# LenShustek/readtape

Hardware: AMD Instinct MI355X
Metric: Msamples/sec (all tracks) 9-trk TBIN (higher is better)
Workload: dtype i16/f32; 1 GPU; C2: synthetic 9-track 800 BPI NRZI, 781.25 kHz, 1 parmset; rows_per_gpu=101799450, rows_total=101799450, bytes_per_gpu=1832390100, parmsets=1

## Files before the change

### readtape_amd/csrc/rtfe_api.hip

```cpp
#include <hip/hip_runtime.h>

#include <limits.h>
#include <math.h>
#include <stdarg.h>
#include <stdio.h>
#include <stdlib.h>
#include <string.h>

#include <mutex>

#include "rt_frontend.h"
#include "rtfe_device.h"

#include "rtfe_sift.hip"
#include "rtfe_kernels.hip"
#include "rtfe_zeros.hip"
#include "rtfe_diffz.hip"
#include "rtfe_ww.hip"
#include "rtfe_gain.hip"
#include "rtfe_dense.hip"
#include "rtfe_pack.hip"
#include "rtfe_csv.hip"

namespace rtfe {
// ... 345 lines not shown
      fprintf(stderr, "rtfe: peak path %d, k_sift LDS %d (halo %d/%d rows, slots %d bytes, %d vectors per thread)\n", d.peak_path, d.pk_lds, d.pk_hl, d.pk_hr, d.pk_slot, sf_nv(d));
      for (int sidx = 0; sidx < d.nscreens; ++sidx) fprintf(stderr, "rtfe: screen %d W %d rise_i %d minpk_i %d sure_i %d\n", sidx, d.screen[sidx].W, d.screen[sidx].rise_i, d.screen[sidx].minpk_i, d.screen[sidx].sure_i); }
   hipDeviceProp_t prop;
   int dev = 0;
   if (hipGetDevice(&dev) != hipSuccess || hipGetDeviceProperties(&prop, dev) != hipSuccess) { delete h; return fail(-20, "no HIP device"); }
   h->num_cus = prop.multiProcessorCount;
   if (hipMalloc(&h->d_dev, sizeof(DevCfg)) != hipSuccess) { delete h; return fail(-21, "hipMalloc failed"); }
   if (hipMemcpy(h->d_dev, &d, sizeof(DevCfg), hipMemcpyHostToDevice) != hipSuccess) { (void)hipFree(h->d_dev); delete h; return fail(-22, "hipMemcpy failed"); }
   raise_dynamic_lds(reinterpret_cast<const void *>(k_decode), h->lds_bytes);
   h->zeros_kernel = getenv("RTFE_ZEROS_KERNEL") ? atoi(getenv("RTFE_ZEROS_KERNEL")) != 0 : 1;
   h->diffz_kernel = getenv("RTFE_DIFFZ_KERNEL") ? atoi(getenv("RTFE_DIFFZ_KERNEL")) != 0 : 1;
   if (!(d.find_zeros && d.differentiate) || d.mode == RTFE_WW) h->diffz_kernel = 0;
   h->side = nullptr; h->overlap = getenv("RTFE_OVERLAP") ? atoi(getenv("RTFE_OVERLAP")) != 0 : 1;
   h->graphs = getenv("RTFE_GRAPHS") ? atoi(getenv("RTFE_GRAPHS")) != 0 : 0;
   memset(h->gcache, 0, sizeof h->gcache); h->gstamp = 0;
   h->bursts_wpr = getenv("RTFE_BURSTS_WPR") ? atoi(getenv("RTFE_BURSTS_WPR")) : 0;
   h->ds_order = getenv("RTFE_DS_ORDER") ? atoi(getenv("RTFE_DS_ORDER")) : 1;
   h->dchain_wgs = getenv("RTFE_DCHAIN_WGS") ? atoi(getenv("RTFE_DCHAIN_WGS")) : 16;
   h->prep_wgs = getenv("RTFE_PREP_WGS") ? atoi(getenv("RTFE_PREP_WGS")) : 32;
   h->prep_run = getenv("RTFE_PREP_RUN") ? atoi(getenv("RTFE_PREP_RUN")) : 8;
   if (h->prep_run < 1 || h->prep_run > kPrepMaxRun) h->prep_run = 8;
   h->work_cap = getenv("RTFE_WORK_CAP") ? atoll(getenv("RTFE_WORK_CAP")) : -1;
   h->ccap_max = getenv("RTFE_CCAP") ? atoll(getenv("RTFE_CCAP")) : 0;
   h->dense_stop = getenv("RTFE_DENSE_STOP") ? atoi(getenv("RTFE_DENSE_STOP")) : 99;
   h->dseg_wgs = getenv("RTFE_DSEG_WGS") ? atoi(getenv("RTFE_DSEG_WGS")) : 0;
   h->dseg_threads = getenv("RTFE_DSEG_THREADS") ? atoi(getenv("RTFE_DSEG_THREADS")) : 0;
   h->seg_cap = getenv("RTFE_SEG_CAP") ? atoll(getenv("RTFE_SEG_CAP")) : 0;
   h->peak_stop = getenv("RTFE_PEAK_STOP") ? atoi(getenv("RTFE_PEAK_STOP")) : 99;
   h->sift_wgs = getenv("RTFE_SIFT_WGS") ? atoi(getenv("RTFE_SIFT_WGS")) : 0;
   h->sift_generic = getenv("RTFE_SIFT_GENERIC") != nullptr;
   h->sift_per_screen = !(getenv("RTFE_SIFT_PER_SCREEN") && atoi(getenv("RTFE_SIFT_PER_SCREEN")) == 0);
   h->dseg_generic = getenv("RTFE_DSEG_GENERIC") != nullptr;
   if (d.invert || d.maxskew > 0 || d.ntrks < 2 || d.zc_peak_i < 1 || d.zc_peak_i > 32767 || !d.zc_parallel) h->zeros_kernel = 0;
   if (d.peak_path) {
      raise_dynamic_lds(reinterpret_cast<const void *>(sf_kernel(sf_wmax(d), sf_threads(d), sf_nv(d))), d.pk_lds);
      for (int sc = 0; sc < kMaxScreens; ++sc) h->sfs_occ[sc] = 0;
      if (sf_special(h)) for (int sc = 0; sc < d.nscreens; ++sc) {
         raise_dynamic_lds(reinterpret_cast<const void *>(sf_special_sc(h, sc)), sfs_lds_sc(d, sc));
         int nb = 0;
         if (hipOccupancyMaxActiveBlocksPerMultiprocessor(&nb, reinterpret_cast<const void *>(sf_special_sc(h, sc)), sfs_threads(d), (size_t)sfs_lds_sc(d, sc)) == hipSuccess && nb >= 1) h->sfs_occ[sc] = nb; } }
   if (d.dense_path) raise_dynamic_lds(reinterpret_cast<const void *>(ds_kernel(h)), (int)ds_lds_layout(d.ntrks, d.halo_rows, d.ds_pad + kDsTile + kDsRight, d.ds_up).total + 64);
   (void)hipGetLastError();
   if (getenv("RTFE_VERBOSE") && d.peak_path) {
      int nb = -1;
      const sfs_kernel_t sfs = sf_special(h);
      const int thr = sfs ? sfs_threads(d) : sf_threads(d), lds = sfs ? sfs_lds(d) : d.pk_lds;
      (void)hipOccupancyMaxActiveBlocksPerMultiprocessor(&nb, sfs ? reinterpret_cast<const void *>(sfs) : reinterpret_cast<const void *>(sf_kernel(sf_wmax(d), sf_threads(d), sf_nv(d))), thr, (size_t)lds);
      fprintf(stderr, "rtfe: k_sift%s %d threads, %d bytes of LDS: %d workgroups per CU (occupancy API), %d CUs\n", sfs ? "_s" : "", thr, lds, nb, h->num_cus); }
   *out = h;
   return 0; }

constexpr int kTimingRing = 64;
static_assert(kTimingRing <= 64, "rtfe_handle::ev_ran holds 64 sets");
static void timing_free(rtfe_handle *h) {
   if (!h->ev0) return;
   for (int r = 0; r < kTimingRing; ++r) for (int i = 0; i < kNumKernels; ++i) { (void)hipEventDestroy(h->ev0[r][i]); (void)hipEventDestroy(h->ev1[r][i]); }
   delete[] h->ev0; delete[] h->ev1; h->ev0 = nullptr; h->ev1 = nullptr; }

extern "C" int rtfe_set_timing(rtfe_handle *h, int enable) {
   if (!h) return fail(-1, "null argument");
   if (enable && !h->timing) {
      h->ev0 = new hipEvent_t[kTimingRing][12]; h->ev1 = new hipEvent_t[kTimingRing][12];
      for (int r = 0; r < kTimingRing; ++r) for (int i = 0; i < kNumKernels; ++i)
      {
         const bool ok0 = hipEventCreate(&h->ev0[r][i]) == hipSuccess;
         const bool ok1 = ok0 && hipEventCreate(&h->ev1[r][i]) == hipSuccess;
         if (!ok1) {
            if (ok0) (void)hipEventDestroy(h->ev0[r][i]);
            for (int r2 = 0; r2 <= r; ++r2) for (int i2 = 0; i2 < (r2 < r ? kNumKernels : i); ++i2) { (void)hipEventDestroy(h->ev0[r2][i2]); (void)hipEventDestroy(h->ev1[r2][i2]); }
            delete[] h->ev0; delete[] h->ev1; h->ev0 = nullptr; h->ev1 = nullptr;
            return fail(-40, "hipEventCreate failed"); } }
      h->ev_next = 0; h->ev_pending = 0; }
   if (!enable && h->timing) timing_free(h);
   h->timing = enable != 0;
   return 0; }

extern "C" int rtfe_kernel_ms(rtfe_handle *h, float *out) {
   if (!h || !out || !h->timing) return fail(-41, "timing is not enabled");
   const int n = h->ev_pending < kTimingRing ? h->ev_pending : kTimingRing;
   for (int i = 0; i < kNumKernels; ++i) out[i] = 0;
   for (int k = 0; k < n; ++k) {
      const int r = ((h->ev_next - 1 - k) % kTimingRing + kTimingRing) % kTimingRing;
      for (int i = 0; i < kNumKernels; ++i) {
         float ms = 0;
         if (hipEventSynchronize(h->ev1[r][i]) != hipSuccess) return fail(-42, "hipEventSynchronize failed");
         if (hipEventElapsedTime(&ms, h->ev0[r][i], h->ev1[r][i]) != hipSuccess) return fail(-43, "hipEventElapsedTime failed");
         if ((h->ev_ran[r] >> i) & 1u) out[i] += ms; } }
   h->ev_pending = 0;
   return n; }

extern "C" void rtfe_destroy(rtfe_handle *h) {
   if (!h) return;
   if (h->timing) timing_free(h);
   drop_graphs(h);
   if (h->side) { (void)hipEventDestroy(h->ev_fork); (void)hipEventDestroy(h->ev_join); (void)hipEventDestroy(h->ev_fork2); (void)hipEventDestroy(h->ev_join2); (void)hipStreamDestroy(h->side); }
   (void)hipFree(h->d_dev);
   delete h; }

extern "C" int rtfe_pkww_width(const rtfe_handle *h, int parmset) {
   return (h && parmset >= 0 && parmset < h->dev.nparm) ? h->dev.parm[parmset].W : -1; }

constexpr int kBrRoundsMax = 1024;

extern "C" int64_t rtfe_max_bursts(const rtfe_handle *h, int64_t nrows) {
   return (nrows / kChunkRows) / h->dev.gap_chunks + 4; }

struct WsLayout {
   long long nwords, max_bursts, ptiles, dtiles;
   long long ccap, seg_cap, work_cap; int hard_cap;
   size_t scratch, qwords, rtot, ctl, dir, chain, pool, hard, ovf, qtile, tstart, crec, eref, extra, cst, segs, gfire, work, dead, slot, total; };

static size_t align256(size_t x) { return (x + 255) & ~(size_t)255; }

static WsLayout ws_layout(const rtfe_handle *h, int64_t nrows) {
   const DevCfg &d = h->dev;
   const bool pk = d.peak_path != 0, ds = d.dense_path != 0;
   const size_t nlists = (size_t)d.nscreens * d.ntrks, nchains = (size_t)d.nparm * d.ntrks;
   WsLayout L;
   L.nwords = ((nrows / kChunkRows + 1) + 63) / 64 + 1;
   L.max_bursts = rtfe_max_bursts(h, nrows);
   L.ptiles = (nrows + kSfTile - 1) / kSfTile;
   L.dtiles = (nrows + kDsTile - 1) / kDsTile;
   L.ccap = L.ptiles * (d.pk_slot / 8 + 1) + 64;
   if (h->ccap_max > 0 && h->ccap_max < L.ccap) L.ccap = h->ccap_max;
   const long long sift_wgs = L.ptiles < (long long)h->num_cus * 8 ? L.ptiles : (long long)h->num_cus * 8;
   const long long hard = L.ptiles * d.nscreens * d.ntrks * 2 + 4096 + sift_wgs * 4 * kSfHardChunk * d.nscreens;
   L.hard_cap = (int)(hard > 0x3fffffffll ? 0x3fffffffll : hard);
   L.seg_cap = 0;
   if (pk) L.seg_cap = h->seg_cap >= 1 ? h->seg_cap
                                       : (L.ccap / d.pk_seg_recs + 1) * d.nscreens * d.ntrks * (d.nparm < 2 ? 1 : 2) + L.max_bursts * d.nparm * d.ntrks + 64;
   size_t off = 0;
   auto take = [&off](bool on, size_t bytes) { const size_t at = off; if (on) off = align256(off + bytes); return at; };
   L.scratch = 0;
   L.qwords = kScratchBytes;
   L.rtot = L.qwords + (size_t)L.nwords * 8;
   off = align256(L.rtot + (size_t)kBrRoundsMax * 4);
   L.ctl = take(true, (size_t)L.max_bursts * sizeof(BurstCtl));
   L.dir = take(pk, (size_t)(L.ptiles + 1) * nlists * sizeof(PeakDir));
   L.chain = take(pk, (size_t)L.max_bursts * nchains * sizeof(float));
   L.pool = take(pk, (size_t)L.ptiles * nlists * (size_t)d.pk_slot);
   L.hard = take(pk, (size_t)L.hard_cap * sizeof(SfHard));
   L.ovf = take(pk, (size_t)L.hard_cap * kSfOvfBytes);
   L.qtile = take(pk, (size_t)L.ptiles * 2);
   L.tstart = take(pk, ((size_t)L.ptiles + 2 * ((size_t)(L.ptiles + 1023) / 1024) + 2) * nlists * 4);
   L.crec = take(pk, (size_t)L.ccap * nlists * sizeof(CRec));
   L.eref = take(pk, (size_t)L.ccap * nlists * 8);
   L.extra = take(pk, (size_t)L.ptiles * nlists * 4);
   L.cst = take(pk, (size_t)L.max_bursts * nchains * sizeof(ChainSt));
   L.segs = take(pk, (size_t)L.seg_cap * sizeof(GsSeg));
   L.gfire = take(pk, (size_t)L.seg_cap * (size_t)(d.pk_seg_recs > 0 ? d.pk_seg_recs : 0) * 4);
   L.work = L.gfire;
   L.work_cap = (long long)((off - L.gfire) / 8);
   if (h->work_cap >= 0 && h->work_cap < L.work_cap) L.work_cap = h->work_cap;
   if (L.work_cap > 0x7ffffe00ll) L.work_cap = 0x7ffffe00ll;
   L.dead = take(ds, (size_t)L.dtiles * d.nscreens);
   L.slot = take(ds, (size_t)L.dtiles * kDsJ * d.nuset * d.ntrks * (size_t)d.ds_slot + 256);
   L.total = off + 256;
   return L; }

extern "C" size_t rtfe_workspace_bytes(const rtfe_handle *h, int64_t nrows) { return ws_layout(h, nrows).total; }

extern "C" int64_t rtfe_event_capacity(const rtfe_handle *h, int64_t nrows) {
   const double per_track = (double)nrows * h->dev.cap_frac + 128.0 * (double)rtfe_max_bursts(h, nrows) + (double)kMarginRows;
   return (int64_t)(per_track * h->dev.nparm * h->dev.ntrks) + 4096; }

struct WsView {
   BurstScratch *scratch; unsigned long long *qwords; uint32_t *rtot; BurstCtl *ctl;
   PeakDir *dir; float *chain; unsigned char *pool; SfHard *hard; unsigned char *ovf; uint16_t *qtile;
   uint32_t *tstart, *ctotc, *coff, *ctot;
   CRec *crec; uint2 *eref; int *extra; ChainSt *cst; GsSeg *segs; float *gfire; unsigned long long *work;
   unsigned char *dead, *slot; };

template <class T> static T *ws_at(void *ws, size_t off) { return reinterpret_cast<T *>(static_cast<char *>(ws) + off); }

static WsView ws_view(const rtfe_handle *h, const WsLayout &L, void *ws) {
   WsView w;
   w.scratch = ws_at<BurstScratch>(ws, L.scratch); w.qwords = ws_at<unsigned long long>(ws, L.qwords); w.rtot = ws_at<uint32_t>(ws, L.rtot); w.ctl = ws_at<BurstCtl>(ws, L.ctl);
   w.dir = ws_at<PeakDir>(ws, L.dir); w.chain = ws_at<float>(ws, L.chain); w.pool = ws_at<unsigned char>(ws, L.pool); w.hard = ws_at<SfHard>(ws, L.hard);
   w.ovf = ws_at<unsigned char>(ws, L.ovf); w.qtile = ws_at<uint16_t>(ws, L.qtile);
   const size_t nlists = h->dev.peak_path ? (size_t)h->dev.nscreens * h->dev.ntrks : 0, nsc = (size_t)(L.ptiles + 1023) / 1024;
   w.tstart = ws_at<uint32_t>(ws, L.tstart); w.ctotc = w.tstart + (size_t)L.ptiles * nlists; w.coff = w.ctotc + nsc * nlists; w.ctot = w.coff + nsc * nlists;
   w.crec = ws_at<CRec>(ws, L.crec); w.eref = ws_at<uint2>(ws, L.eref); w.extra = ws_at<int>(ws, L.extra); w.cst = ws_at<ChainSt>(ws, L.cst);
   w.segs = ws_at<GsSeg>(ws, L.segs); w.gfire = ws_at<float>(ws, L.gfire); w.work = ws_at<unsigned long long>(ws, L.work);
   w.dead = ws_at<unsigned char>(ws, L.dead); w.slot = ws_at<unsigned char>(ws, L.slot);
   return w; }

static int launch_check(const char *what) {
   hipError_t e = hipGetLastError();
   if (e != hipSuccess) return fail(-30, "%s: %s", what, hipGetErrorString(e));
   return 0; }

static void ensure_side(rtfe_handle *h) {
   if (h->side || !h->overlap) return;
   int pr_least = 0, pr_greatest = 0;
   (void)hipDeviceGetStreamPriorityRange(&pr_least, &pr_greatest);
   if (hipStreamCreateWithPriority(&h->side, hipStreamNonBlocking, pr_greatest) != hipSuccess) { (void)hipGetLastError(); h->side = nullptr; h->overlap = 0; }
   else { (void)hipEventCreateWithFlags(&h->ev_fork, hipEventDisableTiming); (void)hipEventCreateWithFlags(&h->ev_join, hipEventDisableTiming);
          (void)hipEventCreateWithFlags(&h->ev_fork2, hipEventDisableTiming); (void)hipEventCreateWithFlags(&h->ev_join2, hipEventDisableTiming); } }

struct ScanArgs {
   const int16_t *d_rows; int64_t nrows, own_rows, row_base; int first_is_tape_start;
   void *d_workspace; size_t workspace_bytes;
   rtfe_burst *d_bursts; int64_t max_bursts; int32_t *d_nbursts;
   uint32_t *d_counts; rtfe_event *d_events; int64_t event_capacity; void *stream; };

static void graph_key(const ScanArgs &a, unsigned long long key[13]) {
   auto u = [](auto v) { return (unsigned long long)(uintptr_t)v; };
   const unsigned long long k[13] = {u(a.d_rows), u(a.nrows), u(a.own_rows), u(a.row_base), u(a.first_is_tape_start), u(a.d_workspace), u(a.workspace_bytes),
                                     u(a.d_bursts), u(a.max_bursts), u(a.d_nbursts), u(a.d_counts), u(a.d_events), u(a.event_capacity)};
   memcpy(key, k, sizeof k); }

struct Scan {
   rtfe_handle *h; const DevCfg &d; const ScanArgs &a; hipStream_t st; WsLayout L; WsView w;
   long long nrows, row_base, nchunks, maxb;
   int evset; bool ran[kNumKernels];
   void t0s(int k, hipStream_t s) { ran[k] = true; if (h->timing) (void)hipEventRecord(h->ev0[evset][k], s); }
   void t1s(int k, hipStream_t s) { if (h->timing) (void)hipEventRecord(h->ev1[evset][k], s); }
   void t0(int k) { t0s(k, st); }
   void t1(int k) { t1s(k, st); }
   void skip_rest() {
      unsigned mask = 0;
      for (int k = 0; k < kNumKernels; ++k) if (ran[k]) mask |= 1u << k;
      if (h->timing) h->ev_ran[evset] = mask;
      for (int k = 0; k < kNumKernels; ++k) if (!ran[k]) { t0(k); t1(k); } }
   void launch_bursts(hipStream_t s) {
      const int wpr_env = h->bursts_wpr;
      const int wpr = (wpr_env >= 1 && wpr_env <= kBrWords) ? wpr_env : kBrWords;
      const long long rounds = (L.nwords + wpr - 1) / wpr;
      if ((wpr_env > 0 || rounds >= 3) && rounds <= kBrRoundsMax && d.debug != 5) {
         hipLaunchKernelGGL(k_bursts_cnt, dim3((unsigned)rounds), dim3(1024), 0, s, (const unsigned long long *)w.qwords, L.nwords, nchunks, wpr, d.gap_chunks, a.first_is_tape_start, maxb, w.rtot);
         hipLaunchKernelGGL(k_bursts_emit, dim3((unsigned)rounds), dim3(1024), 0, s, (const unsigned long long *)w.qwords, L.nwords, nchunks, nrows, wpr, d.gap_chunks, a.first_is_tape_start, a.d_bursts, maxb, (const uint32_t *)w.rtot);
         hipLaunchKernelGGL(k_bursts_tail, dim3(1), dim3(1024), 0, s, (int)rounds, (const uint32_t *)w.rtot, nrows, (long long)a.own_rows, d.ntrks, d.gap_chunks,
                            d.cap_frac, d.nparm, (long long)a.event_capacity, a.d_bursts, maxb, w.scratch, a.d_nbursts); }
      else
         hipLaunchKernelGGL(k_bursts, dim3(1), dim3(1024), 0, s, (const unsigned long long *)w.qwords, L.nwords, nchunks, nrows, (long long)a.own_rows, d.ntrks,
                            d.gap_chunks, a.first_is_tape_start, d.cap_frac, d.nparm, (long long)a.event_capacity, a.d_bursts, maxb, w.scratch, a.d_nbursts, d.debug == 5 ? 1 : 0); }
   void launch_zones(hipStream_t s) {
      hipLaunchKernelGGL(k_zones, dim3(h->num_cus * 8), dim3(64), 0, s, h->d_dev, a.d_rows, nrows, (const rtfe_burst *)a.d_bursts, (const BurstScratch *)w.scratch, w.ctl);
      if (d.invert)
         hipLaunchKernelGGL(k_rails, dim3(h->num_cus * 8), dim3(64), 0, s, h->d_dev, a.d_rows, nrows, (const rtfe_burst *)a.d_bursts, (const BurstScratch *)w.scratch, w.ctl); }
   void launch_decode(int mode) {
      const DecodePlan dp = decode_plan(h);
      t0(kTDecode);
      hipLaunchKernelGGL(k_decode, dim3(h->num_cus * dp.per_cu), dim3(dp.threads), h->lds_bytes, st, h->d_dev, a.d_rows, nrows,
                         row_base, a.d_bursts, w.scratch, a.d_counts, a.d_events, 0xffffffffu, 0, 0, mode, w.ctl);
      t1(kTDecode); }
   void launch_sift() {
      t0(kTSift);
      const sfs_kernel_t sfs = sf_special(h);
      const int pthreads = sfs ? sfs_threads(d) : sf_threads(d), plds = sfs ? sfs_lds(d) : d.pk_lds;
      int spc = lds_wgs_per_cu(plds, 512, 32 / (pthreads / 64));
      if (h->sift_wgs >= 1 && h->sift_wgs < spc) spc = h->sift_wgs;
      if (spc < 1) spc = 1;
      long long pgrid = (long long)h->num_cus * spc;
      if (pgrid > L.ptiles) pgrid = L.ptiles;
      if (sfs) {
         for (int sc = 0; sc < d.nscreens; ++sc) {
            SfArgs sa;
            sa.rows = a.d_rows; sa.nrows = nrows; sa.ntiles = (int)L.ptiles; sa.qtile = sc == 0 ? w.qtile : nullptr; sa.dir = w.dir; sa.pool = w.pool; sa.hard = w.hard; sa.hard_cap = L.hard_cap;
            sa.hard_count = &w.scratch->hard_count; sa.dbg = w.scratch->scr; sa.hcap = d.pk_slot; sa.wave_cap = d.pk_wave_cap; sa.invert = d.invert;
            sa.quiet_i = d.quiet_i; sa.cfg = h->d_dev; sa.hi_i = d.screen[sc].sure_i;
            sa.cut = d.cut; sa.debug = d.debug; sa.defer = 1; sa.nscreens = d.nscreens; sa.sc = sc;
            const int lds_sc = sfs_lds_sc(d, sc);
            int spc_sc = lds_wgs_per_cu(lds_sc, 512, spc);
            if (h->sfs_occ[sc] >= 1 && spc_sc > h->sfs_occ[sc]) spc_sc = h->sfs_occ[sc];
            if (spc_sc < 1) spc_sc = 1;
            long long grid_sc = (long long)h->num_cus * spc_sc;
            if (grid_sc > L.ptiles) grid_sc = L.ptiles;
            hipLaunchKernelGGL(sf_special_sc(h, sc), dim3((unsigned)grid_sc), dim3(pthreads), lds_sc, st, sa); } }
      else {
         const sf_kernel_t sfk = sf_kernel(sf_wmax(d), pthreads, sf_nv(d));
         hipLaunchKernelGGL(sfk, dim3((unsigned)pgrid), dim3(pthreads), d.pk_lds, st, (const DevCfg *)h->d_dev, a.d_rows, nrows, L.ptiles,
                            w.qtile, w.dir, w.pool, w.hard, L.hard_cap, &w.scratch->hard_count, w.scratch->scr); }
      t1(kTSift); }
   void launch_streams() {
      t0(kTPrep);
      const int nlists = d.nscreens * d.ntrks;
      const int nsc = (int)((L.ptiles + 1023) / 1024);
      hipLaunchKernelGGL(k_sift_hard, dim3(h->num_cus * 16), dim3(256), 0, st, (const DevCfg *)h->d_dev, a.d_rows, nrows, (const SfHard *)w.hard, L.hard_cap,
                         (const int *)&w.scratch->hard_count, w.ovf, w.extra, w.scratch->dbg2);
      hipLaunchKernelGGL(k_pscan1, dim3(nsc), dim3(1024), 0, st, (const PeakDir *)w.dir, (const int *)w.extra, (int)L.ptiles, nlists, w.tstart, w.ctotc);
      hipLaunchKernelGGL(k_pscan2, dim3(1), dim3(1024), 0, st, nsc, nlists, (const uint32_t *)w.ctotc, w.coff, w.ctot);
      PrepArgs ppa; ppa.nlists = nlists; ppa.ntrks = d.ntrks; ppa.hcap = d.pk_slot; ppa.run = h->prep_run; ppa.mv = d.maxvolts;
      hipLaunchKernelGGL(k_prep, dim3(h->num_cus * (h->prep_wgs >= 1 && h->prep_wgs <= 4096 ? h->prep_wgs : 32)), dim3(256), 0, st, ppa, (const PeakDir *)w.dir, (const unsigned char *)w.pool, (const unsigned char *)w.ovf,
                         (const uint32_t *)w.tstart, (const uint32_t *)w.coff, (const uint32_t *)w.ctot, L.ptiles, L.ccap, w.crec, w.eref, w.work, L.work_cap, &w.scratch->prep_work);
      hipLaunchKernelGGL(k_clear, dim3(h->num_cus * 4), dim3(256), 0, st, (const unsigned long long *)w.work, L.work_cap, (const int *)&w.scratch->prep_work, (const uint32_t *)w.ctot, L.ccap, w.crec);
#ifdef RTFE_CPU_EMUL
      if (getenv("RTFE_PREP_CHECK")) hipLaunchKernelGGL(k_prep_check, dim3(1), dim3(64), 0, st, (const DevCfg *)h->d_dev, (const uint32_t *)w.ctot, L.ccap, (const CRec *)w.crec);
      if (getenv("RTFE_PREP_CHECK") && atoi(getenv("RTFE_PREP_CHECK")) > 1)
         hipLaunchKernelGGL(k_prep_shapes, dim3(1), dim3(64), 0, st, nlists, (int)d.pk_slot, h->prep_run, L.ptiles, L.ccap, (const PeakDir *)w.dir, (const unsigned char *)w.pool, (const uint32_t *)w.ctot);
#endif
      t1(kTPrep); }
   void launch_chains() {
      t0(kTGain);
      for (int mode = 0; mode < 2; ++mode) {
         if (mode == 1) t0(kTGainTail);
         hipLaunchKernelGGL(k_gain, dim3(h->num_cus * 4), dim3(64), 0, st, (const DevCfg *)h->d_dev, mode, w.cst, nrows, row_base, (const rtfe_burst *)a.d_bursts,
                            w.scratch, w.ctl, a.d_counts, a.d_events, w.chain, (const CRec *)w.crec, (const uint2 *)w.eref, (const uint32_t *)w.tstart, (const uint32_t *)w.coff, (const uint32_t *)w.ctot, L.ccap,
                            (const unsigned char *)w.pool, L.ptiles, w.segs, L.seg_cap, a.d_rows);
         if (mode == 0) {
            t1(kTGain); t0(kTGainS);
            hipLaunchKernelGGL(k_gain_seg, dim3(h->num_cus * 16), dim3(64), 0, st, (const DevCfg *)h->d_dev, (const ChainSt *)w.cst, w.scratch, (const CRec *)w.crec, L.ccap, w.segs, (const int *)&w.scratch->nsegs, L.seg_cap, w.gfire);
            hipLaunchKernelGGL(k_gain_join, dim3(h->num_cus * 2), dim3(64), 0, st, (const DevCfg *)h->d_dev, w.cst, (const rtfe_burst *)a.d_bursts, w.scratch, (const BurstCtl *)w.ctl, a.d_counts, w.chain, w.segs);
            t1(kTGainS); } }
#ifdef RTFE_CPU_EMUL
      if (getenv("RTFE_PREP_CHECK") && atoi(getenv("RTFE_PREP_CHECK")) > 1 && d.pk_seg_recs > 0)
         hipLaunchKernelGGL(k_seg_shapes, dim3(1), dim3(64), 0, st, (const DevCfg *)h->d_dev, (const ChainSt *)w.cst, (const BurstScratch *)w.scratch, (const CRec *)w.crec, L.ccap,
                            (const GsSeg *)w.segs, L.seg_cap, (const float *)w.gfire);
#endif
      t1(kTGainTail); }
   void launch_emit(hipStream_t side) {
      t0(kTEmit);
      hipStream_t se = st;
      if (side != st) { se = side; (void)hipEventRecord(h->ev_fork2, st); (void)hipStreamWaitEvent(se, h->ev_fork2, 0); }
      hipLaunchKernelGGL(k_emit, dim3(h->num_cus * 32), dim3(64), 0, se, h->d_dev, (const rtfe_burst *)a.d_bursts, (const BurstScratch *)w.scratch, (const BurstCtl *)w.ctl, (const uint32_t *)a.d_counts, a.d_events,
// ... 322 lines not shown
```

### readtape_amd/csrc/rtfe_kernels.hip

```cpp
#include <hip/hip_runtime.h>
#include <stdint.h>

#include "rtfe_device.h"

namespace rtfe {

constexpr int kScratchBytes = 512;
struct BurstScratch {
   int   nbursts;
   int   queue;
   int   nbursts_total;
   int   queue_walk;
   int   queue_resume;
   int   queue_seg, nsegs;
   int   queue_stitch;
   int   seg_failed;
   int   hard_count;
   int   min_height_key;
   float floor_used;
   int   prep_work;
   int   pad[3];
   unsigned long long dbg[8];
   unsigned long long pool_cursor;
   unsigned long long dbg2[8];
// ... 22 lines not shown

__global__ void k_adapt_floor(DevCfg *cfg, const BurstScratch *scratch) {
   if (threadIdx.x != 0 || blockIdx.x != 0 || !cfg->adapt_floor || cfg->differentiate || cfg->find_zeros) return;
   const int key = scratch->min_height_key;
   if (key <= 0) return;
   cfg->floor_probed = 1;
   float want = 0.5f * __uint_as_float((unsigned)(0x7fffffff - key));
   if (want > 4.0f) want = 4.0f;
   if (want < cfg->floor_cfg) want = cfg->floor_cfg;
   if (want == cfg->floor_now) return;
   screen_thresholds(*cfg, want); }

__global__ void k_reset_floor(DevCfg *cfg) {
   if (threadIdx.x != 0 || blockIdx.x != 0) return;
   cfg->floor_probed = 0; cfg->probe_min = 0x7fffffff; cfg->probe_ticket = 0;
   if (cfg->floor_now != cfg->floor_cfg) screen_thresholds(*cfg, cfg->floor_cfg); }

constexpr int kProbeRows = 512, kProbeWindows = 4096;
__global__ void __launch_bounds__(256) k_scan_begin(DevCfg *cfg, BurstScratch *scratch, uint4 *extra, long long extra_vecs, const int16_t *__restrict__ rows, long long nrows) {
   __shared__ int s_mx[RTFE_MAXTRKS], s_mn[RTFE_MAXTRKS];
   __shared__ unsigned int s_noisy;
   const int tid = threadIdx.x;
   for (long long v = (long long)blockIdx.x * 256 + tid; v < extra_vecs; v += (long long)gridDim.x * 256) extra[v] = make_uint4(0, 0, 0, 0);
   if (blockIdx.x == 0) for (int i = tid; i < kScratchBytes / 4; i += 256) reinterpret_cast<int *>(scratch)[i] = 0;
   const bool probe = cfg->adapt_floor && !cfg->floor_probed && cfg->probe_on && !cfg->differentiate && !cfg->find_zeros && nrows >= 4 * kChunkRows;
   if (!probe) {
      __syncthreads();
      if (blockIdx.x == 0 && tid == 0) scratch->floor_used = cfg->floor_now;
      return; }
   const int ntrks = cfg->ntrks, q = cfg->quiet_i;
   const long long nwin = nrows / kProbeRows < 1 ? 1 : (nrows / kProbeRows > kProbeWindows ? kProbeWindows : nrows / kProbeRows);
   const int nstr = 256 / ntrks, trk = tid % ntrks, rg = tid / ntrks;
   for (long long w = blockIdx.x; w < nwin; w += gridDim.x) {
      const long long r0 = ((w * nrows) / nwin) & ~63ll;
      const int len = (int)(nrows - r0 < kProbeRows ? nrows - r0 : kProbeRows);
      if (tid < ntrks) { s_mx[tid] = -0x10000; s_mn[tid] = 0x10000; }
      if (tid == 0) s_noisy = 0;
      __syncthreads();
      if (rg < nstr) {
         int mx = -0x10000, mn = 0x10000;
         unsigned int loud = 0;
         const int16_t *col = rows + r0 * ntrks + trk;
         for (int i = rg; i < len; i += nstr) {
            const int x = col[(long long)i * ntrks];
            mx = x > mx ? x : mx; mn = x < mn ? x : mn;
            if (x > q || x < -q) loud |= 1u << (i >> 6); }
         atomicMax(&s_mx[trk], mx); atomicMin(&s_mn[trk], mn);
         if (loud) atomicOr(&s_noisy, loud); }
      __syncthreads();
      if (tid == 0) {
         const int ngroups = len >> 6;
         const unsigned all = (1u << ngroups) - 1u;
         if (ngroups >= 4 && (s_noisy & all) == all) {
            int est = 0x7fffffff;
            for (int t = 0; t < ntrks; ++t) if (s_mx[t] > q && s_mn[t] < -q && s_mx[t] - s_mn[t] < est) est = s_mx[t] - s_mn[t];
            if (est != 0x7fffffff) atomicMin(&cfg->probe_min, est); } }
      __syncthreads(); }
   __syncthreads();
   if (tid != 0) return;
   __threadfence();
   if (atomicAdd(&cfg->probe_ticket, 1u) != gridDim.x - 1) return;
   __threadfence();
   const int m = atomicMin(&cfg->probe_min, 0x7fffffff);
   cfg->probe_min = 0x7fffffff; cfg->probe_ticket = 0;
   if (m != 0x7fffffff) {
      cfg->floor_probed = 1;
      float want = 0.45f * ((float)m / 32767.0f * cfg->maxvolts);
      if (want > 4.0f) want = 4.0f;
      if (want < cfg->floor_cfg) want = cfg->floor_cfg;
      if (want != cfg->floor_now) screen_thresholds(*cfg, want); }
   scratch->floor_used = cfg->floor_now; }

__device__ __forceinline__ bool quiet_at(const u64 *q, long long c, long long nchunks) {
   return c >= 0 && c < nchunks && ((q[c >> 6] >> (c & 63)) & 1); }

__device__ __forceinline__ int block_excl_scan_1024(int v, int *lds, int *total) {
   const int lane = threadIdx.x & 63, wave = threadIdx.x >> 6;
   int x = v;
   #pragma unroll
   for (int o = 1; o < 64; o <<= 1) { int y = __shfl_up(x, o); if (lane >= o) x += y; }
   if (lane == 63) lds[wave] = x;
   __syncthreads();
   if (threadIdx.x == 0) { int s = 0; for (int i = 0; i < 16; ++i) { int t = lds[i]; lds[i] = s; s += t; } lds[16] = s; }
   __syncthreads();
   const int r = x - v + lds[wave];
   *total = lds[16];
   __syncthreads();
   return r; }

constexpr int kBrPer = 4;
constexpr int kBrWords = 1024 * kBrPer;
constexpr int kBrBack = 64, kBrWin = kBrBack + kBrWords + 1;
struct BrWin {
   const u64 *qwords; long long nwords, nchunks, wbase; const u64 *s_q;
   __device__ __forceinline__ u64 qword(long long w) const {
      if (w < 0 || w >= nwords) return 0;
      const long long k = w - wbase;
      return (k >= 0 && k < kBrWin) ? s_q[k] : qwords[w]; }
   __device__ __forceinline__ bool quiet(long long c) const { return c >= 0 && c < nchunks && ((qword(c >> 6) >> (c & 63)) & 1); } };
__device__ __forceinline__ BrWin br_window(const u64 *__restrict__ qwords, long long nwords, long long nchunks, long long w0, u64 *s_q) {
   BrWin bw; bw.qwords = qwords; bw.nwords = nwords; bw.nchunks = nchunks; bw.wbase = w0 - kBrBack; bw.s_q = s_q;
   __syncthreads();
   {  u64 t[(kBrWin + 1023) / 1024];
      #pragma unroll
      for (int j = 0; j < (kBrWin + 1023) / 1024; ++j) { const long long w = bw.wbase + j * 1024 + (int)threadIdx.x; t[j] = (w >= 0 && w < nwords) ? qwords[w] : 0; }
      #pragma unroll
      for (int j = 0; j < (kBrWin + 1023) / 1024; ++j) { const int k = j * 1024 + (int)threadIdx.x; if (k < kBrWin) s_q[k] = t[j]; } }
   __syncthreads();
   return bw; }
__device__ __forceinline__ bool br_exact_start(const BrWin &bw, int gap_chunks, int first_is_start, long long max_bursts) {
   bool starts_quiet = true;
   for (int c = 0; c < gap_chunks; ++c) if (!bw.quiet(c)) { starts_quiet = false; break; }
   return first_is_start && !starts_quiet && max_bursts > 0; }
__device__ __forceinline__ int br_ends(const BrWin &bw, long long w0, int wpr, int gap_chunks, u64 (&ends)[kBrPer]) {
   int cnt = 0;
   #pragma unroll
   for (int j = 0; j < kBrPer; ++j) {
      const int wi = (int)threadIdx.x * kBrPer + j;
      const long long w = w0 + wi;
      ends[j] = 0;
      if (wi < wpr && w < bw.nwords) {
         const u64 q = bw.s_q[kBrBack + wi];
         const u64 qn = bw.s_q[kBrBack + wi + 1];
         const u64 next = (q >> 1) | (qn << 63);
         u64 cand = q & ~next;
         const u64 qp = bw.s_q[kBrBack + wi - 1];
         while (cand) {
            const int bit = __ffsll((long long)cand) - 1;
            cand &= cand - 1;
            bool ok = true;
            if (gap_chunks <= 64) {
               const u64 v = bit == 63 ? q : ((q << (63 - bit)) | (qp >> (bit + 1)));
               ok = ((~v) >> (64 - gap_chunks)) == 0; }
            else {
               const long long c = w * 64 + bit;
               for (int k = 1; k < gap_chunks; ++k) if (!bw.quiet(c - k)) { ok = false; break; } }
            if (ok) ends[j] |= 1ull << bit; } }
      cnt += __popcll(ends[j]); }
   return cnt; }
__device__ __forceinline__ void br_emit(const BrWin &bw, long long w0, const u64 (&ends)[kBrPer], long long idx0, long long nrows, rtfe_burst *__restrict__ bursts, long long max_bursts) {
   long long idx = idx0;
   #pragma unroll
   for (int j = 0; j < kBrPer; ++j) {
      const long long w = w0 + (long long)threadIdx.x * kBrPer + j;
      u64 e = ends[j];
      while (e) {
         const int bit = __ffsll((long long)e) - 1;
         e &= e - 1;
         const long long c1 = w * 64 + bit + 1;
         long long c0 = c1 - 1;
         for (;;) {
            if (c0 == 0) break;
            const long long pw = (c0 - 1) >> 6; const int pb = (int)((c0 - 1) & 63);
            const u64 run = ~(bw.qword(pw) << (63 - pb));
            const int ones = run ? __clzll((long long)run) : 64;
            const int take = ones < pb + 1 ? ones : pb + 1;
            c0 -= take;
            if (take < pb + 1) break; }
         if (idx < max_bursts) {
            rtfe_burst b = {};
            long long zf = c0 * kChunkRows;
            long long ze = c1 * kChunkRows;
            if (ze > nrows) ze = nrows & ~63ll;
            b.zone_first = zf; b.zone_end = ze; b.reset_sample = -1; b.safe_last = -1;
            bursts[idx] = b; }
         ++idx; } } }
__device__ __forceinline__ void br_tail(int nb_found, long long nrows, long long own_rows, int ntrks, int gap_chunks, float cap_frac, int nparm, long long event_capacity,
                                        rtfe_burst *__restrict__ bursts, long long max_bursts, BurstScratch *__restrict__ scratch, int32_t *__restrict__ nbursts_out, int *lds) {
   __shared__ u64 s_ebase;
   __shared__ int s_owned;
   int nb = nb_found;
   if (nb > max_bursts) nb = (int)max_bursts;
   if (threadIdx.x == 0) s_owned = nb;
   __syncthreads();
   for (int b0 = 0; b0 < nb; b0 += 1024) {
      const int b = b0 + threadIdx.x;
      if (b < nb && own_rows < nrows && bursts[b].zone_end >= own_rows + (long long)gap_chunks * kChunkRows && !(bursts[b].flags & RTFE_F_EXACT_START)) atomicMin(&s_owned, b); }
   __syncthreads();
   const int n_owned = s_owned;
   if (nb > n_owned + 1) nb = n_owned + 1;
   if (threadIdx.x == 0) s_ebase = 0;
   __syncthreads();
   for (int b0 = 0; b0 < nb; b0 += 1024) {
      const int b = b0 + threadIdx.x;
      long long cap = 0;
      if (b < nb) {
         const long long start = (bursts[b].flags & RTFE_F_EXACT_START) ? 0 : bursts[b].zone_end - kMarginRows;
         const long long end = (b + 1 < nb) ? bursts[b + 1].zone_end : nrows;
         long long len = end - start;
         if (len < 0) len = 0;
         cap = (long long)((float)len * cap_frac) + 64;
         bursts[b].end_sample = end;
         bursts[b].event_cap = (uint32_t)cap; }
      int total;
      const int units = (int)((cap * nparm * ntrks + 63) >> 6);
      const int eoff = block_excl_scan_1024(units, lds, &total);
      if (b < nb) {
         const u64 base = s_ebase + ((u64)eoff << 6);
         if ((long long)(base + (u64)cap * nparm * ntrks) > event_capacity) {
            bursts[b].event_cap = 0; bursts[b].flags |= RTFE_F_EVENT_OVERFLOW; }
         bursts[b].event_base = base; }
      __syncthreads();
      if (threadIdx.x == 0) s_ebase += (u64)total << 6;
      __syncthreads(); }
   if (threadIdx.x == 0) {
      scratch->nbursts = n_owned; scratch->nbursts_total = nb; scratch->queue = 0; scratch->queue_walk = 0; scratch->queue_resume = 0; scratch->queue_seg = 0; scratch->nsegs = 0; scratch->queue_stitch = 0; scratch->seg_failed = 0; *nbursts_out = n_owned;
      if (n_owned == nb && own_rows < nrows && n_owned > 0) bursts[n_owned - 1].flags |= RTFE_F_TRUNCATED; }
   if (threadIdx.x < 8) scratch->dbg[threadIdx.x] = 0;
   if (threadIdx.x >= 16 && threadIdx.x < 24) scratch->dbg2[threadIdx.x - 16] = 0;
   if (threadIdx.x >= 24 && threadIdx.x < 32) scratch->why[threadIdx.x - 24] = 0; }

__global__ void __launch_bounds__(1024) k_bursts(const u64 *__restrict__ qwords, long long nwords, long long nchunks,
                                                 long long nrows, long long own_rows, int ntrks, int gap_chunks, int first_is_start,
                                                 float cap_frac, int nparm, long long event_capacity,
                                                 rtfe_burst *__restrict__ bursts, long long max_bursts,
                                                 BurstScratch *__restrict__ scratch, int32_t *__restrict__ nbursts_out, int prof) {
   __shared__ int lds[32];
   long long pk0 = prof ? clock64() : 0, pk1 = 0, pk2 = 0;
   __shared__ int s_base;
   __shared__ u64 s_q[kBrWin];
   if (threadIdx.x == 0) s_base = 0;
   for (long long w0 = 0; w0 < nwords; w0 += kBrWords) {
      const BrWin bw = br_window(qwords, nwords, nchunks, w0, s_q);
      if (w0 == 0 && threadIdx.x == 0 && br_exact_start(bw, gap_chunks, first_is_start, max_bursts)) {
         rtfe_burst b = {};
         b.zone_first = 0; b.zone_end = 0; b.reset_sample = 0; b.safe_last = 0; b.flags = RTFE_F_EXACT_START;
         bursts[0] = b;
         s_base = 1; }
      __syncthreads();
      u64 ends[kBrPer];
      const int cnt = br_ends(bw, w0, kBrWords, gap_chunks, ends);
      int total;
      const int off = block_excl_scan_1024(cnt, lds, &total);
      const int base = s_base;
      br_emit(bw, w0, ends, (long long)base + off, nrows, bursts, max_bursts);
      __syncthreads();
      if (threadIdx.x == 0) s_base = base + total; }
   __syncthreads();
   if (prof) pk1 = clock64();
   br_tail(s_base, nrows, own_rows, ntrks, gap_chunks, cap_frac, nparm, event_capacity, bursts, max_bursts, scratch, nbursts_out, lds);
   if (prof && threadIdx.x == 0) { pk2 = clock64(); scratch->scr[0] = (unsigned long long)(pk1 - pk0); scratch->scr[1] = (unsigned long long)(pk2 - pk1); }
   }

__global__ void __launch_bounds__(1024) k_bursts_cnt(const u64 *__restrict__ qwords, long long nwords, long long nchunks, int wpr, int gap_chunks, int first_is_start,
                                                     long long max_bursts, uint32_t *__restrict__ rtot) {
   __shared__ int lds[32];
   __shared__ u64 s_q[kBrWin];
   const long long w0 = (long long)blockIdx.x * wpr;
   const BrWin bw = br_window(qwords, nwords, nchunks, w0, s_q);
   u64 ends[kBrPer];
   const int cnt = br_ends(bw, w0, wpr, gap_chunks, ends);
   int total;
   (void)block_excl_scan_1024(cnt, lds, &total);
   if (threadIdx.x == 0) rtot[blockIdx.x] = (uint32_t)total + ((blockIdx.x == 0 && br_exact_start(bw, gap_chunks, first_is_start, max_bursts)) ? 1u : 0u); }
__global__ void __launch_bounds__(1024) k_bursts_emit(const u64 *__restrict__ qwords, long long nwords, long long nchunks, long long nrows, int wpr, int gap_chunks, int first_is_start,
                                                      rtfe_burst *__restrict__ bursts, long long max_bursts, const uint32_t *__restrict__ rtot) {
   __shared__ int lds[32];
   __shared__ u64 s_q[kBrWin];
   const long long w0 = (long long)blockIdx.x * wpr;
   long long base;
   {  long long mine = 0;
      for (int r = threadIdx.x; r < (int)blockIdx.x; r += 1024) mine += rtot[r];
      int total;
      (void)block_excl_scan_1024((int)(mine > 0x3fffffll ? 0x3fffffll : mine), lds, &total);
      base = total; }
   const BrWin bw = br_window(qwords, nwords, nchunks, w0, s_q);
   if (blockIdx.x == 0 && br_exact_start(bw, gap_chunks, first_is_start, max_bursts)) {
      if (threadIdx.x == 0) {
         rtfe_burst b = {};
         b.zone_first = 0; b.zone_end = 0; b.reset_sample = 0; b.safe_last = 0; b.flags = RTFE_F_EXACT_START;
         bursts[0] = b; }
      base = 1; }
   u64 ends[kBrPer];
   const int cnt = br_ends(bw, w0, wpr, gap_chunks, ends);
   int total;
   const int off = block_excl_scan_1024(cnt, lds, &total);
   br_emit(bw, w0, ends, base + off, nrows, bursts, max_bursts); }
__global__ void __launch_bounds__(1024) k_bursts_tail(int nrounds, const uint32_t *__restrict__ rtot, long long nrows, long long own_rows, int ntrks, int gap_chunks,
                                                      float cap_frac, int nparm, long long event_capacity, rtfe_burst *__restrict__ bursts, long long max_bursts,
                                                      BurstScratch *__restrict__ scratch, int32_t *__restrict__ nbursts_out) {
   __shared__ int lds[32];
   long long mine = 0;
   for (int r = threadIdx.x; r < nrounds; r += 1024) mine += rtot[r];
   int total;
   (void)block_excl_scan_1024((int)(mine > 0x3fffffll ? 0x3fffffll : mine), lds, &total);
   br_tail(total, nrows, own_rows, ntrks, gap_chunks, cap_frac, nparm, event_capacity, bursts, max_bursts, scratch, nbursts_out, lds); }

struct Tile {
   int16_t *x;
   int      halo;
   int      ldw;
   const int *colof;
   long long row0;
   int      nrows;
   long long reset;
   unsigned char *bits;
   int      bstride;
   unsigned char *ldpos;
   int      ldstride;
   int      ntrks;
   const int *skew;
   float   *fd;
   int      rail;
   __device__ __forceinline__ float fy(int t, long long n) const {
      const int d = skew[t];
      const long long m = (n - reset < d) ? n : n - d;
      return fd[((int)(m - row0) + halo) * ntrks + colof[t]]; }
   __device__ __forceinline__ int xi(int t, long long n) const { const int v = x[((int)(n - row0) + halo) * ntrks + colof[t]]; return v == rail ? 32768 : v; }
   __device__ __forceinline__ int y(int t, long long n) const {
      const int d = skew[t];
      return xi(t, (n - reset < d) ? n : n - d); }
   __device__ __forceinline__ unsigned char *ldmap(int screen, int kind, int t) const {
      return ldpos + (screen * 2 + kind) * (ntrks * ldstride) + t * ldstride + kScreenHalo; }
   __device__ __forceinline__ const u64 *map(int screen, int kind, int t) const {
      return reinterpret_cast<const u64 *>(bits + (screen * 5 + kind) * (ntrks * bstride) + t * bstride + kScreenHalo / 8); }
};

struct Col {
   const int16_t *p; int P;
   __device__ __forceinline__ int operator[](int i) const { return p[i * P]; } };
__device__ __forceinline__ Col tile_col(const Tile &tl, int trk, int delay) {
   Col c; c.P = tl.ntrks; c.p = tl.x + (tl.halo - delay) * tl.ntrks + tl.colof[trk]; return c; }
#ifdef RTFE_CPU_EMUL
typedef const int16_t *gptr16;
#else
typedef const __attribute__((address_space(1))) int16_t *gptr16;
#endif
struct GCol {
   gptr16 base; int off, P;
   __device__ __forceinline__ int operator[](int i) const {
#ifdef RTFE_CPU_EMUL
      return base[off + i * P];
#else
      return *(gptr16)((const __attribute__((address_space(1))) char *)base + (unsigned)((off + i * P) << 1));
#endif
   } };
template <bool kGlobal> __device__ __forceinline__ auto zc_col(const Tile &tl, int trk, int delay) {
   if constexpr (kGlobal) { GCol g; g.base = (gptr16)tl.x; g.off = (tl.halo - delay) * tl.ntrks + tl.colof[trk]; g.P = tl.ntrks; return g; }
   else return tile_col(tl, trk, delay); }

__device__ __forceinline__ float volt(int i, float maxvolts) {
   return (float)i / 32767 * maxvolts; }
__device__ __forceinline__ int zc_rail(const DevCfg *cfg) { return cfg->invert ? -32768 : (1 << 30); }
__device__ __forceinline__ int zc_code(int v, int rail) { return v == rail ? 32768 : v; }

struct Walker {
   long long start;
   long long next;
   long long blind_until;
   int   minv;
   long long qtrig;
   long long cpos;
   bool  chain_pending;
   int   slow_max, slow_countdown;
   bool  fast;
   long long trust_from;
   float agc_gain, v_avg_height, v_avg_height_sum;
   int   v_avg_height_count, peakcount, heightndx;
   float v_top, v_bot, v_lasttop, v_lastbot;
   int   z_prev, z_top, z_bot;
   float zf_top, zf_bot, zf_lastraw;
   long long z_firstzero, z_lastzero;
   bool  z_up_pending, z_dn_pending;
   long long z_ttop_row, z_tbot_row;
   bool  datablock, bit1_up;
   double t_lastpeak;
   float rise, reqmin;
   bool  thr_dirty;
// ... 1038 lines not shown
```

Baseline: 81210 Msamples/s.

## Restructure burst tail pass to process eight bursts per thread with 256 threads

Rewrites the single-block burst tail kernel so each thread handles eight consecutive bursts in registers, fusing the ownership scan and event-capacity allocation into one pass. A block-size-generic exclusive scan is added and the kernel is launched with 256 threads instead of 1024, cutting barrier and scan rounds. Timing bookkeeping also stops recording dummy events for kernels that did not run. This targets the latency of a serial single-block stage. In exchange, ownership is now resolved per round, which may differ subtly from the prior whole-array atomicMin.

```diff
diff --git a/readtape_amd/csrc/rtfe_api.hip b/readtape_amd/csrc/rtfe_api.hip
--- a/readtape_amd/csrc/rtfe_api.hip
+++ b/readtape_amd/csrc/rtfe_api.hip
@@ -451,10 +451,11 @@
    for (int k = 0; k < n; ++k) {
       const int r = ((h->ev_next - 1 - k) % kTimingRing + kTimingRing) % kTimingRing;
       for (int i = 0; i < kNumKernels; ++i) {
+         if (!((h->ev_ran[r] >> i) & 1u)) continue;
          float ms = 0;
          if (hipEventSynchronize(h->ev1[r][i]) != hipSuccess) return fail(-42, "hipEventSynchronize failed");
          if (hipEventElapsedTime(&ms, h->ev0[r][i], h->ev1[r][i]) != hipSuccess) return fail(-43, "hipEventElapsedTime failed");
-         if ((h->ev_ran[r] >> i) & 1u) out[i] += ms; } }
+         out[i] += ms; } }
    h->ev_pending = 0;
    return n; }
 
@@ -590,8 +591,7 @@
    void skip_rest() {
       unsigned mask = 0;
       for (int k = 0; k < kNumKernels; ++k) if (ran[k]) mask |= 1u << k;
-      if (h->timing) h->ev_ran[evset] = mask;
-      for (int k = 0; k < kNumKernels; ++k) if (!ran[k]) { t0(k); t1(k); } }
+      if (h->timing) h->ev_ran[evset] = mask; }
    void launch_bursts(hipStream_t s) {
       const int wpr_env = h->bursts_wpr;
       const int wpr = (wpr_env >= 1 && wpr_env <= kBrWords) ? wpr_env : kBrWords;
@@ -599,7 +599,7 @@
       if ((wpr_env > 0 || rounds >= 3) && rounds <= kBrRoundsMax && d.debug != 5) {
          hipLaunchKernelGGL(k_bursts_cnt, dim3((unsigned)rounds), dim3(1024), 0, s, (const unsigned long long *)w.qwords, L.nwords, nchunks, wpr, d.gap_chunks, a.first_is_tape_start, maxb, w.rtot);
          hipLaunchKernelGGL(k_bursts_emit, dim3((unsigned)rounds), dim3(1024), 0, s, (const unsigned long long *)w.qwords, L.nwords, nchunks, nrows, wpr, d.gap_chunks, a.first_is_tape_start, a.d_bursts, maxb, (const uint32_t *)w.rtot);
-         hipLaunchKernelGGL(k_bursts_tail, dim3(1), dim3(1024), 0, s, (int)rounds, (const uint32_t *)w.rtot, nrows, (long long)a.own_rows, d.ntrks, d.gap_chunks,
+         hipLaunchKernelGGL(k_bursts_tail, dim3(1), dim3(kBtThreads), 0, s, (int)rounds, (const uint32_t *)w.rtot, nrows, (long long)a.own_rows, d.ntrks, d.gap_chunks,
                             d.cap_frac, d.nparm, (long long)a.event_capacity, a.d_bursts, maxb, w.scratch, a.d_nbursts); }
       else
          hipLaunchKernelGGL(k_bursts, dim3(1), dim3(1024), 0, s, (const unsigned long long *)w.qwords, L.nwords, nchunks, nrows, (long long)a.own_rows, d.ntrks,
diff --git a/readtape_amd/csrc/rtfe_kernels.hip b/readtape_amd/csrc/rtfe_kernels.hip
--- a/readtape_amd/csrc/rtfe_kernels.hip
+++ b/readtape_amd/csrc/rtfe_kernels.hip
@@ -128,6 +128,20 @@
    if (lane == 63) lds[wave] = x;
    __syncthreads();
    if (threadIdx.x == 0) { int s = 0; for (int i = 0; i < 16; ++i) { int t = lds[i]; lds[i] = s; s += t; } lds[16] = s; }
+   __syncthreads();
+   const int r = x - v + lds[wave];
+   *total = lds[16];
+   __syncthreads();
+   return r; }
+
+__device__ __forceinline__ int block_excl_scan(int v, int *lds, int *total) {
+   const int lane = threadIdx.x & 63, wave = threadIdx.x >> 6, nw = (int)blockDim.x >> 6;
+   int x = v;
+   #pragma unroll
+   for (int o = 1; o < 64; o <<= 1) { int y = __shfl_up(x, o); if (lane >= o) x += y; }
+   if (lane == 63) lds[wave] = x;
+   __syncthreads();
+   if (threadIdx.x == 0) { int s = 0; for (int i = 0; i < nw; ++i) { int t = lds[i]; lds[i] = s; s += t; } lds[16] = s; }
    __syncthreads();
    const int r = x - v + lds[wave];
    *total = lds[16];
@@ -211,43 +225,66 @@
             b.zone_first = zf; b.zone_end = ze; b.reset_sample = -1; b.safe_last = -1;
             bursts[idx] = b; }
          ++idx; } } }
+constexpr int kBtPer = 8;
 __device__ __forceinline__ void br_tail(int nb_found, long long nrows, long long own_rows, int ntrks, int gap_chunks, float cap_frac, int nparm, long long event_capacity,
                                         rtfe_burst *__restrict__ bursts, long long max_bursts, BurstScratch *__restrict__ scratch, int32_t *__restrict__ nbursts_out, int *lds) {
    __shared__ u64 s_ebase;
    __shared__ int s_owned;
    int nb = nb_found;
    if (nb > max_bursts) nb = (int)max_bursts;
-   if (threadIdx.x == 0) s_owned = nb;
-   __syncthreads();
-   for (int b0 = 0; b0 < nb; b0 += 1024) {
-      const int b = b0 + threadIdx.x;
-      if (b < nb && own_rows < nrows && bursts[b].zone_end >= own_rows + (long long)gap_chunks * kChunkRows && !(bursts[b].flags & RTFE_F_EXACT_START)) atomicMin(&s_owned, b); }
-   __syncthreads();
-   const int n_owned = s_owned;
-   if (nb > n_owned + 1) nb = n_owned + 1;
-   if (threadIdx.x == 0) s_ebase = 0;
-   __syncthreads();
-   for (int b0 = 0; b0 < nb; b0 += 1024) {
-      const int b = b0 + threadIdx.x;
-      long long cap = 0;
-      if (b < nb) {
-         const long long start = (bursts[b].flags & RTFE_F_EXACT_START) ? 0 : bursts[b].zone_end - kMarginRows;
-         const long long end = (b + 1 < nb) ? bursts[b + 1].zone_end : nrows;
-         long long len = end - start;
-         if (len < 0) len = 0;
-         cap = (long long)((float)len * cap_frac) + 64;
-         bursts[b].end_sample = end;
-         bursts[b].event_cap = (uint32_t)cap; }
+   const int nb_all = nb;
+   const bool shard = own_rows < nrows;
+   const long long cut_row = own_rows + (long long)gap_chunks * kChunkRows;
+   if (threadIdx.x == 0) { s_owned = nb; s_ebase = 0; }
+   __syncthreads();
+   int n_owned = nb;
+   const int per_round = (int)blockDim.x * kBtPer;
+   for (int b0 = 0; b0 < nb; b0 += per_round) {
+      const int f = b0 + (int)threadIdx.x * kBtPer;
+      long long ze[kBtPer + 1];
+      uint32_t fl[kBtPer];
+      #pragma unroll
+      for (int j = 0; j <= kBtPer; ++j) ze[j] = f + j < nb_all ? bursts[f + j].zone_end : 0;
+      #pragma unroll
+      for (int j = 0; j < kBtPer; ++j) fl[j] = f + j < nb_all ? bursts[f + j].flags : 0;
+      if (shard) {
+         int first = -1;
+         #pragma unroll
+         for (int j = kBtPer - 1; j >= 0; --j) if (f + j < nb && ze[j] >= cut_row && !(fl[j] & RTFE_F_EXACT_START)) first = f + j;
+         if (first >= 0) atomicMin(&s_owned, first); }
+      __syncthreads();
+      n_owned = s_owned;
+      if (nb > n_owned + 1) nb = n_owned + 1;
+      long long cap[kBtPer];
+      int units[kBtPer], mine = 0;
+      #pragma unroll
+      for (int j = 0; j < kBtPer; ++j) {
+         const int b = f + j;
+         cap[j] = 0;
+         if (b < nb) {
+            const long long start = (fl[j] & RTFE_F_EXACT_START) ? 0 : ze[j] - kMarginRows;
+            const long long end = (b + 1 < nb) ? ze[j + 1] : nrows;
+            long long len = end - start;
+            if (len < 0) len = 0;
+            cap[j] = (long long)((float)len * cap_frac) + 64; }
+         units[j] = (int)((cap[j] * nparm * ntrks + 63) >> 6);
+         mine += units[j]; }
       int total;
-      const int units = (int)((cap * nparm * ntrks + 63) >> 6);
-      const int eoff = block_excl_scan_1024(units, lds, &total);
-      if (b < nb) {
-         const u64 base = s_ebase + ((u64)eoff << 6);
-         if ((long long)(base + (u64)cap * nparm * ntrks) > event_capacity) {
-            bursts[b].event_cap = 0; bursts[b].flags |= RTFE_F_EVENT_OVERFLOW; }
-         bursts[b].event_base = base; }
+      int eoff = block_excl_scan(mine, lds, &total);
+      const u64 ebase = s_ebase;
+      #pragma unroll
+      for (int j = 0; j < kBtPer; ++j) {
+         const int b = f + j;
+         if (b < nb) {
+            const u64 base = ebase + ((u64)eoff << 6);
+            uint32_t ecap = (uint32_t)cap[j];
+            if ((long long)(base + (u64)cap[j] * nparm * ntrks) > event_capacity) { ecap = 0; bursts[b].flags = fl[j] | RTFE_F_EVENT_OVERFLOW; }
+            bursts[b].end_sample = (b + 1 < nb) ? ze[j + 1] : nrows;
+            bursts[b].event_cap = ecap;
+            bursts[b].event_base = base; }
+         eoff += units[j]; }
       __syncthreads();
-      if (threadIdx.x == 0) s_ebase += (u64)total << 6;
+      if (threadIdx.x == 0) s_ebase = ebase + ((u64)total << 6);
       __syncthreads(); }
    if (threadIdx.x == 0) {
       scratch->nbursts = n_owned; scratch->nbursts_total = nb; scratch->queue = 0; scratch->queue_walk = 0; scratch->queue_resume = 0; scratch->queue_seg = 0; scratch->nsegs = 0; scratch->queue_stitch = 0; scratch->seg_failed = 0; *nbursts_out = n_owned;
@@ -322,14 +359,15 @@
    int total;
    const int off = block_excl_scan_1024(cnt, lds, &total);
    br_emit(bw, w0, ends, base + off, nrows, bursts, max_bursts); }
-__global__ void __launch_bounds__(1024) k_bursts_tail(int nrounds, const uint32_t *__restrict__ rtot, long long nrows, long long own_rows, int ntrks, int gap_chunks,
-                                                      float cap_frac, int nparm, long long event_capacity, rtfe_burst *__restrict__ bursts, long long max_bursts,
-                                                      BurstScratch *__restrict__ scratch, int32_t *__restrict__ nbursts_out) {
+constexpr int kBtThreads = 256;
+__global__ void __launch_bounds__(kBtThreads) k_bursts_tail(int nrounds, const uint32_t *__restrict__ rtot, long long nrows, long long own_rows, int ntrks, int gap_chunks,
+                                                            float cap_frac, int nparm, long long event_capacity, rtfe_burst *__restrict__ bursts, long long max_bursts,
+                                                            BurstScratch *__restrict__ scratch, int32_t *__restrict__ nbursts_out) {
    __shared__ int lds[32];
    long long mine = 0;
-   for (int r = threadIdx.x; r < nrounds; r += 1024) mine += rtot[r];
+   for (int r = threadIdx.x; r < nrounds; r += (int)blockDim.x) mine += rtot[r];
    int total;
-   (void)block_excl_scan_1024((int)(mine > 0x3fffffll ? 0x3fffffll : mine), lds, &total);
+   (void)block_excl_scan((int)(mine > 0x3fffffll ? 0x3fffffll : mine), lds, &total);
    br_tail(total, nrows, own_rows, ntrks, gap_chunks, cap_frac, nparm, event_capacity, bursts, max_bursts, scratch, nbursts_out, lds); }
 
 struct Tile {
```

Result: slower. 79140 Msamples/s (-2.6%).
